# auniquesun/PPT

Measured on AMD Instinct MI355X. Metric: point-clouds/sec fwd+bwd, PointBERT 1024-pt ModelNet40, higher is better.
Workload: dtype f16; 1 GPU; C2: ModelNet40 1024-pt PointBERT (ULIP_PointBERT head_type=0, frozen backbone + PromptLearner), train-mode BN + DropPath, fwd + CE(ls 0.2) + bwd + AdamW; feed=resident, per_gpu_batch=32, global_batch=32, npoints=1024, classes=40, parallelism=dp1

## Files before the change

### include/ppt_hip.h

```cpp
#ifndef PPT_HIP_H
#define PPT_HIP_H

#include <stddef.h>
#include <stdint.h>

#ifdef __cplusplus
extern "C" {
#endif

#define PPT_OK 0
#define PPT_EINVAL (-1)
#define PPT_ELAUNCH (-2)
#define PPT_EUNSUPPORTED (-3)

#define PPT_F32 0
#define PPT_BF16 1
#define PPT_F16 2

const char *ppt_strerror(int code);
int ppt_abi_version(void);

int ppt_fps_f32(const float *xyz, int B, int N, int M, const int64_t *start, int64_t *out_idx,
                float *out_xyz, void *stream);

// ... 170 lines not shown
int ppt_text_mlp_retile_split(const float *W1, const float *W2, void *W1_tiled, void *W2_tiled, int b_pow2, void *stream);
int ppt_text_mlp_pair(const ppt_text_mlp_params *p, void *stream);

typedef struct ppt_text_lin_params {
    const void *A; int64_t lda;
    const void *W;
    const float *bias;
    const float *residual; int64_t ld_res;
    float *C; int64_t ldc;
    int M, N, K;
    int split_a_pow2, split_b_pow2; unsigned int *split_overflow;
    int wave_prio;
} ppt_text_lin_params;
int ppt_text_lin_retile_split(const float *W, void *W_tiled, int N, int K, int b_pow2, void *stream);
int ppt_text_lin_split(const ppt_text_lin_params *p, void *stream);

int ppt_attention_fwd(const void *qkv, void *out, float *lse, int Bt, int T, int H, int hd,
                      float scale, int causal, int dtype, void *stream);
int ppt_attention_bwd(const void *qkv, const void *out, const void *dout, const float *lse,
                      float *delta, void *dqkv, int Bt, int T, int H, int hd, float scale,
                      int causal, int dtype, void *stream);

size_t ppt_attention_prefix_workspace_bytes(int C, int P, int H, int hd);
int ppt_attention_fwd_split16(const void *qkv, void *out, float *lse, int Bt, int T, int P, int H, int hd, float scale, int causal,
                              void *stream);
int ppt_attention_bwd_split16(const void *qkv, const void *out, const void *dout, const float *lse, float *delta, void *dqkv,
                              float *workspace, int Bt, int T, int P, int H, int hd, float scale, int causal, void *stream);
int ppt_attention_prefix_fwd(const void *qkv, void *out, float *lse, int C, int T, int P, int H, int hd, float scale, int dtype,
                             void *stream);
int ppt_attention_prefix_bwd(const void *qkv, const void *out, const void *dout, const float *lse, float *delta, void *dqkv,
// ... 141 lines not shown
```

### ppt_amd/__init__.py

```python
import os

os.environ.setdefault("GPU_MAX_HW_QUEUES", "8")
```

### ppt_amd/_lib.py

```python
import ctypes
import os

_HERE = os.path.dirname(os.path.abspath(__file__))
LIB_PATH = os.environ.get("PPT_HIP_LIB") or os.path.join(_HERE, "csrc", "libppt_hip.so")
_lib = None

PPT_F32, PPT_BF16, PPT_F16 = 0, 1, 2
A_PLAIN, A_AFFINE_RELU, A_CONV1 = 0, 1, 2
ACT_NONE, ACT_RELU, ACT_GELU, ACT_QUICKGELU = 0, 1, 2, 3

c_void_p, c_int, c_int64, c_float, c_size_t = (ctypes.c_void_p, ctypes.c_int, ctypes.c_int64,
                                               ctypes.c_float, ctypes.c_size_t)


class GemmParams(ctypes.Structure):
    _fields_ = [
        ("A", c_void_p), ("lda", c_int64), ("B", c_void_p), ("ldb", c_int64),
        ("C", c_void_p), ("ldc", c_int64), ("M", c_int), ("N", c_int), ("K", c_int),
        ("dtype", c_int), ("c_dtype", c_int),
        ("a_mode", c_int), ("a_scale", c_void_p), ("a_shift", c_void_p), ("pts", c_void_p),
        ("w1", c_void_p), ("b1", c_void_p),
        ("bias", c_void_p), ("group_add", c_void_p), ("group_rows", c_int), ("act", c_int),
        ("dact_pre", c_void_p), ("ld_dact", c_int64),
        ("row_scale", c_void_p), ("row_scale_rows", c_int),
# ... 5 lines not shown
    ]


class LnLinParams(ctypes.Structure):
    _fields_ = [
        ("x", c_void_p), ("W", c_void_p), ("C", c_void_p), ("ln_w", c_void_p), ("ln_b", c_void_p), ("ln_eps", ctypes.c_float),
        ("bias", c_void_p), ("M", c_int), ("N", c_int), ("K", c_int), ("dtype", c_int), ("slices", c_int),
    ]


class TextLinParams(ctypes.Structure):
    _fields_ = [
        ("A", c_void_p), ("lda", c_int64), ("W", c_void_p), ("bias", c_void_p), ("residual", c_void_p), ("ld_res", c_int64),
        ("C", c_void_p), ("ldc", c_int64), ("M", c_int), ("N", c_int), ("K", c_int),
        ("split_a_pow2", c_int), ("split_b_pow2", c_int), ("split_overflow", c_void_p), ("wave_prio", c_int),
    ]


class TextMlpParams(ctypes.Structure):
    _fields_ = [
        ("A", c_void_p), ("lda", c_int64), ("W1", c_void_p), ("W2", c_void_p), ("b1", c_void_p), ("pre", c_void_p), ("parts", c_void_p),
        ("M", c_int), ("D", c_int), ("hidden", c_int), ("mode", c_int), ("dtype", c_int), ("wave_prio", c_int),
        ("ln_w", c_void_p), ("ln_b", c_void_p), ("ln_eps", ctypes.c_float), ("ln_mean", c_void_p), ("ln_rstd", c_void_p),
        ("split_a_pow2", c_int), ("split_b_pow2", c_int), ("split_overflow", c_void_p),
    ]


class VitMlpParams(ctypes.Structure):
    _fields_ = [
        ("x", c_void_p), ("out", c_void_p), ("W1", c_void_p), ("W2", c_void_p), ("ln_w", c_void_p), ("ln_b", c_void_p),
# ... 52 lines not shown
    "ppt_three_nn_interp_fwd": (c_int, [c_void_p, c_int, c_void_p, c_int, c_void_p, c_void_p, c_int, c_int, c_int, c_void_p, c_int,
                                        c_int, c_void_p, c_void_p]),
    "ppt_scatter_rows_bwd": (c_int, [c_void_p, c_void_p, c_void_p, c_int64, c_int, c_int, c_int, c_int, c_int, c_int, c_void_p,
                                     c_void_p]),
    "ppt_sum_groups": (c_int, [c_void_p, c_int64, c_int, c_int, c_void_p, c_void_p]),
    "ppt_vit_mlp_retile": (c_int, [c_void_p, c_void_p, c_void_p, c_void_p, c_void_p]),
    "ppt_vit_proj_retile": (c_int, [c_void_p, c_void_p, c_void_p]),
    "ppt_vit_mlp_bf16": (c_int, [ctypes.POINTER(VitMlpParams), c_void_p]),
    "ppt_lnlin_retile": (c_int, [c_void_p, c_void_p, c_int, c_void_p]),
    "ppt_lnlin": (c_int, [ctypes.POINTER(LnLinParams), c_void_p]),
    "ppt_text_mlp_retile": (c_int, [c_void_p, c_void_p, c_void_p, c_void_p, c_void_p]),
    "ppt_text_mlp_pair": (c_int, [ctypes.POINTER(TextMlpParams), c_void_p]),
    "ppt_text_mlp_retile_split": (c_int, [c_void_p, c_void_p, c_void_p, c_void_p, c_int, c_void_p]),
    "ppt_text_lin_retile_split": (c_int, [c_void_p, c_void_p, c_int, c_int, c_int, c_void_p]),
    "ppt_text_lin_split": (c_int, [ctypes.POINTER(TextLinParams), c_void_p]),
    "ppt_vit_mlp3_retile": (c_int, [c_void_p, c_void_p, c_void_p, c_void_p, c_void_p]),
    "ppt_vit_mlp3_bf16": (c_int, [ctypes.POINTER(VitMlpParams), c_void_p]),
    "ppt_rowgemm_bf16": (c_int, [ctypes.POINTER(RowGemmParams), c_void_p]),
    "ppt_layernorm_fwd": (c_int, [c_void_p, c_void_p, c_int, c_void_p, c_void_p, c_void_p, c_void_p, c_int,
                                  c_void_p, c_void_p, c_int, c_int, c_float, c_void_p]),
    "ppt_layernorm_bwd": (c_int, [c_void_p, c_void_p, c_void_p, c_void_p, c_void_p, c_void_p, c_int,
                                  c_void_p, c_int, c_void_p, c_void_p, c_int, c_int, c_int, c_void_p]),
    "ppt_layernorm_fwd_sum": (c_int, [c_void_p, c_void_p, c_void_p, c_int, c_void_p, c_void_p, c_void_p, c_void_p, c_int,
                                      c_void_p, c_void_p, c_int, c_int, c_float, c_void_p]),
    "ppt_layernorm_bwd_sum": (c_int, [c_void_p, c_int, c_void_p, c_void_p, c_void_p, c_void_p, c_void_p, c_int,
                                      c_void_p, c_int, c_int, c_int, c_void_p]),
    "ppt_col_sums": (c_int, [c_void_p, c_int, c_int, c_int, c_int64, c_void_p, c_void_p]),
    "ppt_attention_fwd": (c_int, [c_void_p, c_void_p, c_void_p, c_int, c_int, c_int, c_int, c_float, c_int,
                                  c_int, c_void_p]),
    "ppt_attention_bwd": (c_int, [c_void_p, c_void_p, c_void_p, c_void_p, c_void_p, c_void_p, c_int, c_int,
# ... 99 lines not shown
```

### ppt_amd/csrc/text_lin_split.hip

```cpp
#include "ppt_common.h"
#include "gemm_common.h"

namespace {

typedef __attribute__((ext_vector_type(4))) float f32x4_t;

constexpr int KC = 512;
constexpr int RB = 2, R = 16 * RB;
constexpr int AP = 2 * KC + 32;
constexpr int A_BYTES = R * AP;
constexpr int LDS_BYTES = 2 * A_BYTES;
constexpr int K1 = KC / 32;
constexpr int D1 = 4;

__device__ __forceinline__ void lds_barrier_l2()
{
    asm volatile("s_waitcnt lgkmcnt(0)" ::: "memory");
    __builtin_amdgcn_s_barrier();
    asm volatile("" ::: "memory");
}

__device__ __forceinline__ void split4_l(const float (&x)[4], uint2 &H, uint2 &L)
{
    uint32_t h[2], l[2];
#pragma unroll
    for (int q = 0; q < 2; ++q) {
        const _Float16 h0 = (_Float16)x[2 * q], h1 = (_Float16)x[2 * q + 1];
        const ppt_h2 hh = {h0, h1};
        const ppt_h2 ll = {(_Float16)(x[2 * q] - (float)h0), (_Float16)(x[2 * q + 1] - (float)h1)};
        h[q] = __builtin_bit_cast(uint32_t, hh);
        l[q] = __builtin_bit_cast(uint32_t, ll);
    }
    H = make_uint2(h[0], h[1]);
    L = make_uint2(l[0], l[1]);
}

template <int NH>
__global__ __launch_bounds__(512, 2) void text_lin_split_kernel(const ppt_text_lin_params p)
{
    constexpr int SLN = 128 * NH;
    constexpr int WAVE_SLICE = K1 * NH * 2048;
    extern __shared__ __align__(16) unsigned char smem[];
    unsigned char *ai = smem;
    const int lane = threadIdx.x & 63;
    const int w = __builtin_amdgcn_readfirstlane(threadIdx.x >> 6);
    const int l15 = lane & 15, kg = lane >> 4, lo16 = lane * 16;
    PPT_PRIO(p.wave_prio);
    const int nsl = p.N / SLN, nck = p.K / KC;
    const int sc = blockIdx.x % (nsl * nck), s = sc % nsl, c = sc / nsl;
    const int row0 = (blockIdx.x / (nsl * nck)) * R;
    const int nrow = min(R, p.M - row0);
    const float sa = pow2f(p.split_a_pow2), inv = pow2f(-(p.split_a_pow2 + p.split_b_pow2));
    uint32_t over = 0;

    const __amdgpu_buffer_rsrc_t r1 = __builtin_amdgcn_make_buffer_rsrc(const_cast<void *>(p.W), 0, (int)((size_t)p.N * p.K * 4), 0x00020000);
    int o1 = ((c * nsl + s) * 8 + w) * WAVE_SLICE;
    auto next1 = [&](uint4 (&f)[2 * NH]) {
#pragma unroll
        for (int i = 0; i < 2 * NH; ++i) f[i] = __builtin_bit_cast(uint4, __builtin_amdgcn_raw_buffer_load_b128(r1, lo16 + 1024 * i, o1, 0));
        o1 += 2048 * NH;
    };
    uint4 g1[D1][2 * NH];
#pragma unroll
    for (int i = 0; i < D1; ++i) next1(g1[i]);

    {
        const float *A = (const float *)p.A + (size_t)c * KC;
        constexpr int PIECES = R * (KC / 4);
        float4 v[PIECES / 512];
#pragma unroll
        for (int it = 0; it < PIECES / 512; ++it) {
            const int i = threadIdx.x + 512 * it, lr = i / (KC / 4), c4 = i % (KC / 4);
            v[it] = make_float4(0.f, 0.f, 0.f, 0.f);
            if (lr < nrow) v[it] = *reinterpret_cast<const float4 *>(A + (size_t)(row0 + lr) * p.lda + 4 * c4);
        }
#pragma unroll
        for (int it = 0; it < PIECES / 512; ++it) {
            const int i = threadIdx.x + 512 * it, lr = i / (KC / 4), c4 = i % (KC / 4);
            const float x[4] = {split_saturate(v[it].x * sa, over), split_saturate(v[it].y * sa, over),
                                split_saturate(v[it].z * sa, over), split_saturate(v[it].w * sa, over)};
            uint2 H, L;
            split4_l(x, H, L);
            *reinterpret_cast<uint2 *>(ai + lr * AP + 8 * c4) = H;
            *reinterpret_cast<uint2 *>(ai + A_BYTES + lr * AP + 8 * c4) = L;
        }
    }
    const int ncol = SLN * s + 16 * NH * w + 4 * kg;
    float4 bv[NH], rv[RB][NH];
#pragma unroll
    for (int h = 0; h < NH; ++h) {
        bv[h] = p.bias ? *reinterpret_cast<const float4 *>(p.bias + ncol + 16 * h) : make_float4(0.f, 0.f, 0.f, 0.f);
#pragma unroll
        for (int rb = 0; rb < RB; ++rb) {
            const int m = row0 + min(16 * rb + l15, nrow - 1);
            rv[rb][h] = p.residual ? *reinterpret_cast<const float4 *>(p.residual + (size_t)m * p.ld_res + ncol + 16 * h) : make_float4(0.f, 0.f, 0.f, 0.f);
        }
    }
    lds_barrier_l2();

    f32x4_t a1[RB][NH];
#pragma unroll
    for (int rb = 0; rb < RB; ++rb)
#pragma unroll
        for (int h = 0; h < NH; ++h) a1[rb][h] = f32x4_t{0.f, 0.f, 0.f, 0.f};
    {
        const unsigned char *ha = ai + l15 * AP + 16 * kg;
        uint4 fh[2][RB], fl[2][RB];
#pragma unroll
        for (int rb = 0; rb < RB; ++rb) {
            fh[0][rb] = *reinterpret_cast<const uint4 *>(ha + rb * 16 * AP);
            fl[0][rb] = *reinterpret_cast<const uint4 *>(ha + A_BYTES + rb * 16 * AP);
        }
#pragma unroll
        for (int ks = 0; ks < K1; ++ks) {
            if (ks + 1 < K1) {
#pragma unroll
                for (int rb = 0; rb < RB; ++rb) {
                    fh[(ks + 1) & 1][rb] = *reinterpret_cast<const uint4 *>(ha + rb * 16 * AP + 64 * (ks + 1));
                    fl[(ks + 1) & 1][rb] = *reinterpret_cast<const uint4 *>(ha + A_BYTES + rb * 16 * AP + 64 * (ks + 1));
                }
            }
#pragma unroll
            for (int h = 0; h < NH; ++h) {
                const uint4 wh = g1[ks % D1][2 * h], wl = g1[ks % D1][2 * h + 1];
#pragma unroll
                for (int rb = 0; rb < RB; ++rb) {
                    a1[rb][h] = h16<f16_t>::mfma16(wh, fl[ks & 1][rb], a1[rb][h]);
                    a1[rb][h] = h16<f16_t>::mfma16(wl, fh[ks & 1][rb], a1[rb][h]);
                    a1[rb][h] = h16<f16_t>::mfma16(wh, fh[ks & 1][rb], a1[rb][h]);
                }
            }
            if (ks + D1 < K1) next1(g1[ks % D1]);
            __builtin_amdgcn_sched_barrier(0);
        }
    }
    float *C = p.C + (size_t)c * p.M * p.ldc;
#pragma unroll
    for (int rb = 0; rb < RB; ++rb) {
        const int lr = 16 * rb + l15;
        if (lr < nrow) {
#pragma unroll
            for (int h = 0; h < NH; ++h)
                *reinterpret_cast<float4 *>(C + (size_t)(row0 + lr) * p.ldc + ncol + 16 * h) =
                    make_float4(a1[rb][h][0] * inv + bv[h].x + rv[rb][h].x, a1[rb][h][1] * inv + bv[h].y + rv[rb][h].y,
                                a1[rb][h][2] * inv + bv[h].z + rv[rb][h].z, a1[rb][h][3] * inv + bv[h].w + rv[rb][h].w);
        }
    }
    split_report(over, p.split_overflow);
}

template <int NH>
__global__ __launch_bounds__(256) void text_lin_retile_split_kernel(const float *__restrict__ W, unsigned char *__restrict__ Wt, int N, int K, int b_pow2)
{
    constexpr int SLN = 128 * NH;
    const int nsl = N / SLN, nck = K / KC;
    const int i = blockIdx.x * 256 + threadIdx.x;
    if (i >= nck * nsl * 8 * K1 * NH * 64) return;
    const int lane = i & 63, f = (i >> 6) % (K1 * NH), w = (i / (64 * K1 * NH)) & 7, sc = i / (64 * K1 * NH * 8);
    const int s = sc % nsl, c = sc / nsl, ks = f / NH, h = f % NH;
    const int l15 = lane & 15, kg = lane >> 4;
    const float sb = pow2f(b_pow2);
    const float *src = W + (size_t)(SLN * s + 16 * NH * w + 16 * h + l15) * K + KC * c + 32 * ks + 8 * kg;
    uint32_t over = 0;
    const float4 a = *reinterpret_cast<const float4 *>(src), b = *reinterpret_cast<const float4 *>(src + 4);
    const float x0[4] = {split_saturate(a.x * sb, over), split_saturate(a.y * sb, over), split_saturate(a.z * sb, over), split_saturate(a.w * sb, over)};
    const float x1[4] = {split_saturate(b.x * sb, over), split_saturate(b.y * sb, over), split_saturate(b.z * sb, over), split_saturate(b.w * sb, over)};
    uint2 h0, l0, h1, l1;
    split4_l(x0, h0, l0);
    split4_l(x1, h1, l1);
    unsigned char *dst = Wt + (size_t)(sc * 8 + w) * (K1 * NH * 2048) + (size_t)f * 2048 + lane * 16;
    *reinterpret_cast<uint4 *>(dst) = make_uint4(h0.x, h0.y, h1.x, h1.y);
    *reinterpret_cast<uint4 *>(dst + 1024) = make_uint4(l0.x, l0.y, l1.x, l1.y);
}

__host__ int slice_halves(int N) { return N >= 1024 ? 2 : 1; }

}

extern "C" int ppt_text_lin_retile_split(const float *W, void *Wt, int N, int K, int b_pow2, void *stream)
{
    if (!W || !Wt || (((uintptr_t)W | (uintptr_t)Wt) & 15) || abs(b_pow2) > 24) return PPT_EINVAL;
    if (N <= 0 || K <= 0 || K % KC || N % 256) return PPT_EUNSUPPORTED;
    const int pieces = N * (K / 8);
    if (slice_halves(N) == 2)
        hipLaunchKernelGGL(text_lin_retile_split_kernel<2>, dim3((pieces + 255) / 256), dim3(256), 0, ppt_stream(stream), W, (unsigned char *)Wt, N, K, b_pow2);
    else
        hipLaunchKernelGGL(text_lin_retile_split_kernel<1>, dim3((pieces + 255) / 256), dim3(256), 0, ppt_stream(stream), W, (unsigned char *)Wt, N, K, b_pow2);
    PPT_CHECK_LAUNCH();
    return PPT_OK;
}

extern "C" int ppt_text_lin_split(const ppt_text_lin_params *pp, void *stream)
{
    if (!pp) return PPT_EINVAL;
    ppt_text_lin_params p = *pp;
    if (!p.A || !p.W || !p.C || p.M <= 0 || p.N <= 0 || p.K <= 0) return PPT_EINVAL;
    if (p.K % KC || p.N % 256) return PPT_EUNSUPPORTED;
    if (p.lda < p.K || (p.lda % 4) || p.ldc < p.N || (p.ldc % 4) || abs(p.split_a_pow2) > 24 || abs(p.split_b_pow2) > 24) return PPT_EINVAL;
    if (((uintptr_t)p.A | (uintptr_t)p.W | (uintptr_t)p.C | (uintptr_t)p.bias | (uintptr_t)p.residual) & 15) return PPT_EINVAL;
    if (p.residual && (p.ld_res < p.N || (p.ld_res % 4))) return PPT_EINVAL;
    if (p.K > KC && (p.bias || p.residual || p.ldc != p.N)) return PPT_EINVAL;
    if (p.wave_prio == 0) p.wave_prio = ppt_get_wave_priority();
    static const int attrs_once = [] {
        (void)hipFuncSetAttribute((const void *)text_lin_split_kernel<1>, hipFuncAttributeMaxDynamicSharedMemorySize, LDS_BYTES);
        (void)hipFuncSetAttribute((const void *)text_lin_split_kernel<2>, hipFuncAttributeMaxDynamicSharedMemorySize, LDS_BYTES);
        return 0;
    }();
    (void)attrs_once;
    const int nh = slice_halves(p.N);
    const int grid = (p.N / (128 * nh)) * (p.K / KC) * ((p.M + R - 1) / R);
    hipStream_t st = ppt_stream(stream);
    if (nh == 2) hipLaunchKernelGGL((text_lin_split_kernel<2>), dim3(grid), dim3(512), LDS_BYTES, st, p);
    else hipLaunchKernelGGL((text_lin_split_kernel<1>), dim3(grid), dim3(512), LDS_BYTES, st, p);
    PPT_CHECK_LAUNCH();
    return PPT_OK;
}
```

### ppt_amd/engine.py

```python
import os

import torch

from . import ops
from .ops import ACT_GELU, ACT_NONE, ACT_QUICKGELU, A_AFFINE_RELU, A_CONV1

ATTN_SCALE = 64 ** -0.5


class WeightCache:

    def __init__(self, dtype, demoted=None):
        self.dtype = dtype
        self._c = {}
        self.demoted = demoted if demoted is not None else set()

    def get(self, t, kind="w", cols=None, pad_to=None):
        key = (id(t), kind, cols, pad_to)
        ent = self._c.get(key)
        if ent is not None and ent[0] is t and ent[1] == t._version:
            return ent[2]
        with torch.no_grad():
            w = t.detach()
            w = w.reshape(w.shape[0], -1)
# ... 669 lines not shown
TEXT_FUSE_LN = os.environ.get("PPT_TEXT_FUSE_LN", "0") != "0"
TEXT_SPLITK = os.environ.get("PPT_TEXT_SPLITK", "1") != "0"
POINTMLP_FUSED_NORM = os.environ.get("PPT_POINTMLP_FUSED_NORM", "1") != "0"


TEXT_MLP_PAIR = os.environ.get("PPT_TEXT_MLP_PAIR", "1") != "0"
TEXT_MLP_PAIR_LN = os.environ.get("PPT_TEXT_MLP_PAIR_LN", "1") != "0"
TEXT_MLP_PAIR_LAST = os.environ.get("PPT_TEXT_MLP_PAIR_LAST", "1") != "0"
TEXT_MLP_PAIR_SPLIT = os.environ.get("PPT_TEXT_MLP_PAIR_SPLIT", "1") != "0"


TEXT_LIN_SPLIT = os.environ.get("PPT_TEXT_LIN_SPLIT", "1") != "0"


def _text_lin_ok(Ta, width):
    return Ta == torch.float32 and TEXT_LIN_SPLIT and ops.split16_enabled() and width == 512


def _text_lin_tiles(sd, name, wca, transposed=False):
    w = sd[name]
    b = ops.SPLIT16_POW2[1]
    return wca.derived(("text_lin_split", name, transposed, b), (w,),
                       lambda: ops.text_lin_retile_split(wca.get(w, "wt") if transposed else wca.get(w), b))


def _text_mlp_pair_ok(Tm):
    return Tm in ops.HALF or (Tm == torch.float32 and TEXT_MLP_PAIR_SPLIT and ops.split16_enabled())


def _text_mlp_tiles(sd, p, wcm, backward):
    wfc, wpr = sd[p + "mlp.c_fc.weight"], sd[p + "mlp.c_proj.weight"]
    if wcm.dtype == torch.float32:
        b = ops.SPLIT16_POW2[1]
        if backward:
            return wcm.derived(("text_mlp_split_bwd", p, b), (wfc, wpr), lambda: ops.text_mlp_retile_split(wcm.get(wpr, "wt"), wcm.get(wfc, "wt"), b))
        return wcm.derived(("text_mlp_split_fwd", p, b), (wfc, wpr), lambda: ops.text_mlp_retile_split(wcm.get(wfc), wcm.get(wpr), b))
    if backward:
        return wcm.derived(("text_mlp_tiles_bwd", p), (wfc, wpr), lambda: ops.text_mlp_retile(wcm.get(wpr, "wt"), wcm.get(wfc, "wt")))
# ... 29 lines not shown
        M = C * L
        add, add_rows = sd["positional_embedding"], L
        xin = prompts.reshape(M, Wd)
        rows = torch.arange(C, device=dev) * L + eot_pos
    saved = {"layers": []} if save else None
    x = xin if add is None else torch.empty((M, Wd), dtype=torch.float32, device=dev)
    fuse = TEXT_FUSE_LN and T in ops.HALF and Wd in ops.ROWGEMM_K
    wca, wcm = _stage_wc(wc, "text_attn"), _stage_wc(wc, "text_mlp")
    Ta, Tm = wca.dtype, wcm.dtype
    if Ta != T or Tm != T:
        fuse = False

    def stats():
        return (torch.empty((M,), dtype=torch.float32, device=dev), torch.empty((M,), dtype=torch.float32, device=dev)) if save else None
    splitk = TEXT_SPLITK and (T in ops.HALF or ops.split16_enabled()) and Tm == T and not fuse and M <= 4096 and Wd == 512
    lin_split = _text_lin_ok(Ta, Wd) and not fuse
    pending = None
    for i in range(layers):
        p = f"transformer.resblocks.{i}."
        if pending is not None:
            x = torch.empty((M, Wd), dtype=torch.float32, device=dev)
            h, mean1, rstd1 = ops.layernorm_fwd_sum(pending[0], pending[1], pending[2], sd[p + "ln_1.weight"], sd[p + "ln_1.bias"], Ta,
                                                    write_xs=x, save_stats=save)
            pending = None
            if lin_split:
                qkv = ops.text_lin_split(h, _text_lin_tiles(sd, p + "attn.in_proj_weight", wca), bias=sd[p + "attn.in_proj_bias"])
            else:
                qkv = ops.gemm(h, wca.get(sd[p + "attn.in_proj_weight"]), out_dtype=Ta, bias=sd[p + "attn.in_proj_bias"])
        elif fuse and add is None:
            st1 = stats()
            mean1, rstd1 = st1 if save else (None, None)
            qkv = ops.rowgemm(xin, wc.get(sd[p + "attn.in_proj_weight"]), ln=(sd[p + "ln_1.weight"], sd[p + "ln_1.bias"]), ln_stats=st1,
                              bias=sd[p + "attn.in_proj_bias"])
        else:
            h, mean1, rstd1 = ops.layernorm_fwd(xin, sd[p + "ln_1.weight"], sd[p + "ln_1.bias"], Ta, add=add,
                                                add_rows=add_rows, write_xs=x if add is not None else None,
                                                save_stats=save)
            if lin_split:
                qkv = ops.text_lin_split(h, _text_lin_tiles(sd, p + "attn.in_proj_weight", wca), bias=sd[p + "attn.in_proj_bias"])
            else:
                qkv = ops.gemm(h, wca.get(sd[p + "attn.in_proj_weight"]), out_dtype=Ta, bias=sd[p + "attn.in_proj_bias"])
        add, add_rows = None, 0
        if P:
            a, lse = ops.attention_prefix_fwd(qkv, C, L, P, heads, ATTN_SCALE, want_lse=save)
        else:
            a, lse = ops.attention_fwd(qkv, C, L, heads, ATTN_SCALE, True, want_lse=save)
        x_mid = torch.empty_like(x)
        if lin_split:
            ops.text_lin_split(a, _text_lin_tiles(sd, p + "attn.out_proj.weight", wca), bias=sd[p + "attn.out_proj.bias"], residual=x, out=x_mid)
        else:
            ops.gemm(a, wca.get(sd[p + "attn.out_proj.weight"]), out=x_mid, bias=sd[p + "attn.out_proj.bias"], residual=x)
        pre = torch.empty((M, sd[p + "mlp.c_fc.weight"].shape[0]), dtype=Tm, device=dev) if save else None
        pair = (TEXT_MLP_PAIR and splitk and (i + 1 < layers or TEXT_MLP_PAIR_LAST) and _text_mlp_pair_ok(Tm)
                and tuple(sd[p + "mlp.c_fc.weight"].shape) == (2048, 512))
        if pair:
            w1t, w2t = _text_mlp_tiles(sd, p, wcm, False)
            if Tm == torch.float32 and TEXT_MLP_PAIR_LN:
                parts, mean2, rstd2 = ops.text_mlp_pair_split(x_mid, w1t, w2t, bias=sd[p + "mlp.c_fc.bias"], pre=pre,
                                                              ln=(sd[p + "ln_2.weight"], sd[p + "ln_2.bias"]), save_stats=save)
            elif Tm == torch.float32:
                h2, mean2, rstd2 = ops.layernorm_fwd(x_mid, sd[p + "ln_2.weight"], sd[p + "ln_2.bias"], Tm, save_stats=save)
                parts = ops.text_mlp_pair_split(h2, w1t, w2t, bias=sd[p + "mlp.c_fc.bias"], pre=pre)
            elif TEXT_MLP_PAIR_LN:
                parts, mean2, rstd2 = ops.text_mlp_pair(x_mid, w1t, w2t, bias=sd[p + "mlp.c_fc.bias"], pre=pre,
# ... 81 lines not shown
                                           sd[p + "ln_2.weight"], ly["mean2"], ly["rstd2"], g, accumulate=True, copy_dtype=Ta)
            d_pre = None
        else:
            d_pre = ops.gemm(g_t, wcm.get(sd[p + "mlp.c_proj.weight"], "wt"), out_dtype=Tm, act=ACT_QUICKGELU,
                             dact_pre=ly["pre"])
        if d_pre is None:
            pass
        elif splitk:
            _, g_t = ops.layernorm_bwd_sum(ops.gemm_splitk(d_pre, wcm.get(sd[p + "mlp.c_fc.weight"], "wt"), 4), ly["x_mid"],
                                           sd[p + "ln_2.weight"], ly["mean2"], ly["rstd2"], g, accumulate=True, copy_dtype=Ta)
        else:
            d_h2 = ops.gemm(d_pre, wcm.get(sd[p + "mlp.c_fc.weight"], "wt"), out_dtype=torch.float32)
            _, _, _, g_t = ops.layernorm_bwd(d_h2, ly["x_mid"], sd[p + "ln_2.weight"], ly["mean2"], ly["rstd2"], dx=g,
                                             accumulate=True, copy_dtype=Ta)
        if lin_split:
            d_a = ops.text_lin_split(g_t, _text_lin_tiles(sd, p + "attn.out_proj.weight", wca, True))
        else:
            d_a = ops.gemm(g_t, wca.get(sd[p + "attn.out_proj.weight"], "wt"), out_dtype=Ta)
        if P:
            d_qkv = ops.attention_prefix_bwd(ly["qkv"], ly["a"], d_a, ly["lse"], C, L, P, heads, ATTN_SCALE)
        else:
            d_qkv = ops.attention_bwd(ly["qkv"], ly["a"], d_a, ly["lse"], C, L, heads, ATTN_SCALE, True)
        if splitk:
            dparts = (ops.text_lin_split(d_qkv, _text_lin_tiles(sd, p + "attn.in_proj_weight", wca, True)) if lin_split
                      else ops.gemm_splitk(d_qkv, wca.get(sd[p + "attn.in_proj_weight"], "wt"), 3))
            _, g_t = ops.layernorm_bwd_sum(dparts, ly["x"],
                                           sd[p + "ln_1.weight"], ly["mean1"], ly["rstd1"], g, accumulate=True, copy_dtype=Tm)
        else:
            d_h = ops.gemm(d_qkv, wca.get(sd[p + "attn.in_proj_weight"], "wt"), out_dtype=torch.float32)
            _, _, _, g_t = ops.layernorm_bwd(d_h, ly["x"], sd[p + "ln_1.weight"], ly["mean1"], ly["rstd1"], dx=g,
                                             accumulate=True, copy_dtype=Tm)
    if s["rows_mode"]:
        return g
    if S != 1.0:
        g.mul_(1.0 / S)
    if not P and L == s["Lfull"]:
        return g.view(C, L, Wd)
    full = torch.zeros((C, s["Lfull"], Wd), dtype=torch.float32, device=dout.device)
    if P:
# ... 27 lines not shown
```

### ppt_amd/ops.py

```python
import ctypes
import os

import torch

from . import _lib
from ._lib import (ACT_GELU, ACT_NONE, ACT_QUICKGELU, ACT_RELU, A_AFFINE_RELU, A_CONV1, A_PLAIN,
                   PPT_BF16, PPT_F16, PPT_F32, GemmParams, RowGemmParams)
from . import _lib as _libmod

_DT = {torch.float32: PPT_F32, torch.bfloat16: PPT_BF16, torch.float16: PPT_F16}
_TORCH_DT = {PPT_F32: torch.float32, PPT_BF16: torch.bfloat16, PPT_F16: torch.float16}
HALF = (torch.bfloat16, torch.float16)


class KernelProfiler:

    def __init__(self):
        self.records = []
        self.kernels = []
        self.executed = []

    def begin(self, name, work, kernel=None, executed=None):
        ev = torch.cuda.Event(enable_timing=True)
        ev.record(torch.cuda.current_stream())
# ... 404 lines not shown
        p.residual, p.ld_res = _p(residual), residual.stride(-2)
    p.C, p.ldc = _p(out), (N if kc > 1 else out.stride(0))
    p.M, p.N, p.K = M, N, K
    p.split_a_pow2 = SPLIT16_POW2[0] if a_pow2 is None else int(a_pow2)
    p.split_b_pow2 = int(wt.ppt_b_pow2)
    if not torch.cuda.is_current_stream_capturing() or a.device.index in _SPLIT_OVERFLOW:
        p.split_overflow = _p(split16_overflow_counter(a.device))
    if profiler is not None:
        profiler.begin("gemm_f32", 2.0 * M * N * K, "ppt_text_lin_split")
    _lib.check(_lib.lib().ppt_text_lin_split(ctypes.byref(p), _stream()), "ppt_text_lin_split")
    if profiler is not None:
        profiler.end()
    return out


def text_mlp_pair(a, w1t, w2t, *, bias=None, pre=None, backward=False, ln=None, ln_eps=1e-5, save_stats=False):
    M = a.shape[0]
    assert a.dim() == 2 and a.shape[1] == 512 and a.stride(1) == 1 and w1t.dtype in HALF and w2t.dtype == w1t.dtype
    if ln is None:
        assert a.dtype == w1t.dtype
    else:
        assert a.dtype == torch.float32 and not backward
    parts = torch.empty((8, M, 512), dtype=torch.float32, device=a.device)
    p = _lib.TextMlpParams()
    p.A, p.lda, p.W1, p.W2, p.b1, p.pre, p.parts = _p(a), a.stride(0), _p(w1t), _p(w2t), _p(bias), _p(pre), _p(parts)
    p.M, p.D, p.hidden, p.mode, p.dtype = M, 512, 2048, int(bool(backward)), dtype_code(w1t)
    mean = rstd = None
    if ln is not None:
        _chk(ln[0], torch.float32, "ln weight"); _chk(ln[1], torch.float32, "ln bias")
        if save_stats:
# ... 771 lines not shown
```

Baseline: 11850 point-clouds/s.

## Add native half-precision text linear kernel path alongside split-f32 kernel

Generalizes the text-encoder linear kernel with a form template, so f16/bf16 activations and weights run a single MFMA per step. The split-f32 path needs two weight parts and three MFMAs per step. A new retile kernel and wrapper feed this path, and the engine routes half-precision text-encoder QKV and out-projection GEMMs (forward and backward) through it when split-K is active, replacing generic gemm calls. It also freezes the inherited GC heap in forked children. The half path drops split overflow tracking and relies on half-precision accuracy.

```diff
diff --git a/include/ppt_hip.h b/include/ppt_hip.h
--- a/include/ppt_hip.h
+++ b/include/ppt_hip.h
@@ -208,6 +208,19 @@
 } ppt_text_lin_params;
 int ppt_text_lin_retile_split(const float *W, void *W_tiled, int N, int K, int b_pow2, void *stream);
 int ppt_text_lin_split(const ppt_text_lin_params *p, void *stream);
+typedef struct ppt_text_lin16_params {
+    const void *A; int64_t lda;
+    const void *W;
+    const float *bias;
+    const float *residual; int64_t ld_res;
+    void *C; int64_t ldc;
+    int M, N, K;
+    int dtype;
+    int c_dtype;
+    int wave_prio;
+} ppt_text_lin16_params;
+int ppt_text_lin_retile16(const void *W, void *W_tiled, int N, int K, void *stream);
+int ppt_text_lin16(const ppt_text_lin16_params *p, void *stream);
 
 int ppt_attention_fwd(const void *qkv, void *out, float *lse, int Bt, int T, int H, int hd,
                       float scale, int causal, int dtype, void *stream);
diff --git a/ppt_amd/__init__.py b/ppt_amd/__init__.py
--- a/ppt_amd/__init__.py
+++ b/ppt_amd/__init__.py
@@ -1,3 +1,12 @@
 import os
 
 os.environ.setdefault("GPU_MAX_HW_QUEUES", "8")
+
+
+def _freeze_inherited_heap():
+    import gc
+    gc.freeze()
+
+
+if hasattr(os, "register_at_fork"):
+    os.register_at_fork(after_in_child=_freeze_inherited_heap)
diff --git a/ppt_amd/_lib.py b/ppt_amd/_lib.py
--- a/ppt_amd/_lib.py
+++ b/ppt_amd/_lib.py
@@ -43,6 +43,14 @@
         ("A", c_void_p), ("lda", c_int64), ("W", c_void_p), ("bias", c_void_p), ("residual", c_void_p), ("ld_res", c_int64),
         ("C", c_void_p), ("ldc", c_int64), ("M", c_int), ("N", c_int), ("K", c_int),
         ("split_a_pow2", c_int), ("split_b_pow2", c_int), ("split_overflow", c_void_p), ("wave_prio", c_int),
+    ]
+
+
+class TextLin16Params(ctypes.Structure):
+    _fields_ = [
+        ("A", c_void_p), ("lda", c_int64), ("W", c_void_p), ("bias", c_void_p), ("residual", c_void_p), ("ld_res", c_int64),
+        ("C", c_void_p), ("ldc", c_int64), ("M", c_int), ("N", c_int), ("K", c_int), ("dtype", c_int), ("c_dtype", c_int),
+        ("wave_prio", c_int),
     ]
 
 
@@ -125,6 +133,8 @@
     "ppt_text_mlp_retile_split": (c_int, [c_void_p, c_void_p, c_void_p, c_void_p, c_int, c_void_p]),
     "ppt_text_lin_retile_split": (c_int, [c_void_p, c_void_p, c_int, c_int, c_int, c_void_p]),
     "ppt_text_lin_split": (c_int, [ctypes.POINTER(TextLinParams), c_void_p]),
+    "ppt_text_lin_retile16": (c_int, [c_void_p, c_void_p, c_int, c_int, c_void_p]),
+    "ppt_text_lin16": (c_int, [ctypes.POINTER(TextLin16Params), c_void_p]),
     "ppt_vit_mlp3_retile": (c_int, [c_void_p, c_void_p, c_void_p, c_void_p, c_void_p]),
     "ppt_vit_mlp3_bf16": (c_int, [ctypes.POINTER(VitMlpParams), c_void_p]),
     "ppt_rowgemm_bf16": (c_int, [ctypes.POINTER(RowGemmParams), c_void_p]),
diff --git a/ppt_amd/csrc/text_lin_split.hip b/ppt_amd/csrc/text_lin_split.hip
--- a/ppt_amd/csrc/text_lin_split.hip
+++ b/ppt_amd/csrc/text_lin_split.hip
@@ -9,9 +9,32 @@
 constexpr int RB = 2, R = 16 * RB;
 constexpr int AP = 2 * KC + 32;
 constexpr int A_BYTES = R * AP;
-constexpr int LDS_BYTES = 2 * A_BYTES;
 constexpr int K1 = KC / 32;
-constexpr int D1 = 4;
+
+struct LinArgs {
+    const void *A; int64_t lda;
+    const void *W;
+    const float *bias;
+    const float *residual; int64_t ld_res;
+    void *C; int64_t ldc;
+    int M, N, K;
+    int c16;
+    int split_a_pow2, split_b_pow2; unsigned int *split_overflow;
+    int wave_prio;
+};
+
+template <int FORM> struct LinForm {
+    using T = typename std::conditional<FORM == PPT_BF16, bf16_t, f16_t>::type;
+    static constexpr bool SPLIT = false;
+    static constexpr int PARTS = 1;
+    static constexpr int D1 = 8;
+};
+template <> struct LinForm<PPT_F32> {
+    using T = f16_t;
+    static constexpr bool SPLIT = true;
+    static constexpr int PARTS = 2;
+    static constexpr int D1 = 4;
+};
 
 __device__ __forceinline__ void lds_barrier_l2()
 {
@@ -35,11 +58,13 @@
     L = make_uint2(l[0], l[1]);
 }
 
-template <int NH>
-__global__ __launch_bounds__(512, 2) void text_lin_split_kernel(const ppt_text_lin_params p)
-{
-    constexpr int SLN = 128 * NH;
-    constexpr int WAVE_SLICE = K1 * NH * 2048;
+template <int NH, int FORM>
+__global__ __launch_bounds__(512, 2) void text_lin_kernel(const LinArgs p)
+{
+    using F = LinForm<FORM>;
+    using T = typename F::T;
+    constexpr int SLN = 128 * NH, NP = F::PARTS * NH, D1 = F::D1;
+    constexpr int WAVE_SLICE = K1 * NP * 1024;
     extern __shared__ __align__(16) unsigned char smem[];
     unsigned char *ai = smem;
     const int lane = threadIdx.x & 63;
@@ -50,21 +75,32 @@
     const int sc = blockIdx.x % (nsl * nck), s = sc % nsl, c = sc / nsl;
     const int row0 = (blockIdx.x / (nsl * nck)) * R;
     const int nrow = min(R, p.M - row0);
-    const float sa = pow2f(p.split_a_pow2), inv = pow2f(-(p.split_a_pow2 + p.split_b_pow2));
     uint32_t over = 0;
 
-    const __amdgpu_buffer_rsrc_t r1 = __builtin_amdgcn_make_buffer_rsrc(const_cast<void *>(p.W), 0, (int)((size_t)p.N * p.K * 4), 0x00020000);
+    const __amdgpu_buffer_rsrc_t r1 = __builtin_amdgcn_make_buffer_rsrc(const_cast<void *>(p.W), 0, (int)((size_t)p.N * p.K * 2 * F::PARTS), 0x00020000);
     int o1 = ((c * nsl + s) * 8 + w) * WAVE_SLICE;
-    auto next1 = [&](uint4 (&f)[2 * NH]) {
-#pragma unroll
-        for (int i = 0; i < 2 * NH; ++i) f[i] = __builtin_bit_cast(uint4, __builtin_amdgcn_raw_buffer_load_b128(r1, lo16 + 1024 * i, o1, 0));
-        o1 += 2048 * NH;
+    auto next1 = [&](uint4 (&f)[NP]) {
+#pragma unroll
+        for (int i = 0; i < NP; ++i) f[i] = __builtin_bit_cast(uint4, __builtin_amdgcn_raw_buffer_load_b128(r1, lo16 + 1024 * i, o1, 0));
+        o1 += 1024 * NP;
     };
-    uint4 g1[D1][2 * NH];
+    constexpr int PIECES16 = R * (KC / 8);
+    uint4 v16[F::SPLIT ? 1 : PIECES16 / 512];
+    if constexpr (!F::SPLIT) {
+        const uint16_t *A = (const uint16_t *)p.A + (size_t)c * KC;
+#pragma unroll
+        for (int it = 0; it < PIECES16 / 512; ++it) {
+            const int i = threadIdx.x + 512 * it, lr = i / (KC / 8), c8 = i % (KC / 8);
+            v16[it] = make_uint4(0, 0, 0, 0);
+            if (lr < nrow) v16[it] = *reinterpret_cast<const uint4 *>(A + (size_t)(row0 + lr) * p.lda + 8 * c8);
+        }
+    }
+    uint4 g1[D1][NP];
 #pragma unroll
     for (int i = 0; i < D1; ++i) next1(g1[i]);
 
-    {
+    if constexpr (F::SPLIT) {
+        const float sa = pow2f(p.split_a_pow2);
         const float *A = (const float *)p.A + (size_t)c * KC;
         constexpr int PIECES = R * (KC / 4);
         float4 v[PIECES / 512];
@@ -84,6 +120,12 @@
             *reinterpret_cast<uint2 *>(ai + lr * AP + 8 * c4) = H;
             *reinterpret_cast<uint2 *>(ai + A_BYTES + lr * AP + 8 * c4) = L;
         }
+    } else {
+#pragma unroll
+        for (int it = 0; it < PIECES16 / 512; ++it) {
+            const int i = threadIdx.x + 512 * it, lr = i / (KC / 8), c8 = i % (KC / 8);
+            *reinterpret_cast<uint4 *>(ai + lr * AP + 16 * c8) = v16[it];
+        }
     }
     const int ncol = SLN * s + 16 * NH * w + 4 * kg;
     float4 bv[NH], rv[RB][NH];
@@ -109,7 +151,7 @@
 #pragma unroll
         for (int rb = 0; rb < RB; ++rb) {
             fh[0][rb] = *reinterpret_cast<const uint4 *>(ha + rb * 16 * AP);
-            fl[0][rb] = *reinterpret_cast<const uint4 *>(ha + A_BYTES + rb * 16 * AP);
+            if constexpr (F::SPLIT) fl[0][rb] = *reinterpret_cast<const uint4 *>(ha + A_BYTES + rb * 16 * AP);
         }
 #pragma unroll
         for (int ks = 0; ks < K1; ++ks) {
@@ -117,36 +159,51 @@
 #pragma unroll
                 for (int rb = 0; rb < RB; ++rb) {
                     fh[(ks + 1) & 1][rb] = *reinterpret_cast<const uint4 *>(ha + rb * 16 * AP + 64 * (ks + 1));
-                    fl[(ks + 1) & 1][rb] = *reinterpret_cast<const uint4 *>(ha + A_BYTES + rb * 16 * AP + 64 * (ks + 1));
+                    if constexpr (F::SPLIT) fl[(ks + 1) & 1][rb] = *reinterpret_cast<const uint4 *>(ha + A_BYTES + rb * 16 * AP + 64 * (ks + 1));
                 }
             }
 #pragma unroll
             for (int h = 0; h < NH; ++h) {
-                const uint4 wh = g1[ks % D1][2 * h], wl = g1[ks % D1][2 * h + 1];
-#pragma unroll
-                for (int rb = 0; rb < RB; ++rb) {
-                    a1[rb][h] = h16<f16_t>::mfma16(wh, fl[ks & 1][rb], a1[rb][h]);
-                    a1[rb][h] = h16<f16_t>::mfma16(wl, fh[ks & 1][rb], a1[rb][h]);
-                    a1[rb][h] = h16<f16_t>::mfma16(wh, fh[ks & 1][rb], a1[rb][h]);
+                if constexpr (F::SPLIT) {
+                    const uint4 wh = g1[ks % D1][2 * h], wl = g1[ks % D1][2 * h + 1];
+#pragma unroll
+                    for (int rb = 0; rb < RB; ++rb) {
+                        a1[rb][h] = h16<f16_t>::mfma16(wh, fl[ks & 1][rb], a1[rb][h]);
+                        a1[rb][h] = h16<f16_t>::mfma16(wl, fh[ks & 1][rb], a1[rb][h]);
+                        a1[rb][h] = h16<f16_t>::mfma16(wh, fh[ks & 1][rb], a1[rb][h]);
+                    }
+                } else {
+#pragma unroll
+                    for (int rb = 0; rb < RB; ++rb) a1[rb][h] = h16<T>::mfma16(g1[ks % D1][h], fh[ks & 1][rb], a1[rb][h]);
                 }
             }
             if (ks + D1 < K1) next1(g1[ks % D1]);
             __builtin_amdgcn_sched_barrier(0);
         }
     }
-    float *C = p.C + (size_t)c * p.M * p.ldc;
 #pragma unroll
     for (int rb = 0; rb < RB; ++rb) {
         const int lr = 16 * rb + l15;
         if (lr < nrow) {
 #pragma unroll
-            for (int h = 0; h < NH; ++h)
-                *reinterpret_cast<float4 *>(C + (size_t)(row0 + lr) * p.ldc + ncol + 16 * h) =
-                    make_float4(a1[rb][h][0] * inv + bv[h].x + rv[rb][h].x, a1[rb][h][1] * inv + bv[h].y + rv[rb][h].y,
-                                a1[rb][h][2] * inv + bv[h].z + rv[rb][h].z, a1[rb][h][3] * inv + bv[h].w + rv[rb][h].w);
-        }
-    }
-    split_report(over, p.split_overflow);
+            for (int h = 0; h < NH; ++h) {
+                if constexpr (F::SPLIT) {
+                    const float inv = pow2f(-(p.split_a_pow2 + p.split_b_pow2));
+                    float *C = (float *)p.C + (size_t)c * p.M * p.ldc;
+                    *reinterpret_cast<float4 *>(C + (size_t)(row0 + lr) * p.ldc + ncol + 16 * h) =
+                        make_float4(a1[rb][h][0] * inv + bv[h].x + rv[rb][h].x, a1[rb][h][1] * inv + bv[h].y + rv[rb][h].y,
+                                    a1[rb][h][2] * inv + bv[h].z + rv[rb][h].z, a1[rb][h][3] * inv + bv[h].w + rv[rb][h].w);
+                } else {
+                    const float4 v = make_float4(a1[rb][h][0] + bv[h].x + rv[rb][h].x, a1[rb][h][1] + bv[h].y + rv[rb][h].y,
+                                                 a1[rb][h][2] + bv[h].z + rv[rb][h].z, a1[rb][h][3] + bv[h].w + rv[rb][h].w);
+                    const size_t off = (size_t)c * p.M * p.ldc + (size_t)(row0 + lr) * p.ldc + ncol + 16 * h;
+                    if (p.c16) *reinterpret_cast<uint2 *>((uint16_t *)p.C + off) = make_uint2(h16<T>::pack2(v.x, v.y), h16<T>::pack2(v.z, v.w));
+                    else *reinterpret_cast<float4 *>((float *)p.C + off) = v;
+                }
+            }
+        }
+    }
+    if constexpr (F::SPLIT) split_report(over, p.split_overflow);
 }
 
 template <int NH>
@@ -173,7 +230,41 @@
     *reinterpret_cast<uint4 *>(dst + 1024) = make_uint4(l0.x, l0.y, l1.x, l1.y);
 }
 
+template <int NH>
+__global__ __launch_bounds__(256) void text_lin_retile16_kernel(const uint16_t *__restrict__ W, unsigned char *__restrict__ Wt, int N, int K)
+{
+    constexpr int SLN = 128 * NH;
+    const int nsl = N / SLN, nck = K / KC;
+    const int i = blockIdx.x * 256 + threadIdx.x;
+    if (i >= nck * nsl * 8 * K1 * NH * 64) return;
+    const int lane = i & 63, f = (i >> 6) % (K1 * NH), w = (i / (64 * K1 * NH)) & 7, sc = i / (64 * K1 * NH * 8);
+    const int s = sc % nsl, c = sc / nsl, ks = f / NH, h = f % NH;
+    const int l15 = lane & 15, kg = lane >> 4;
+    const uint16_t *src = W + (size_t)(SLN * s + 16 * NH * w + 16 * h + l15) * K + KC * c + 32 * ks + 8 * kg;
+    *reinterpret_cast<uint4 *>(Wt + (size_t)i * 16) = *reinterpret_cast<const uint4 *>(src);
+}
+
 __host__ int slice_halves(int N) { return N >= 1024 ? 2 : 1; }
+
+template <int NH, int FORM>
+void launch(const LinArgs &p, hipStream_t st)
+{
+    constexpr int LDS_BYTES = LinForm<FORM>::PARTS * A_BYTES;
+    static const int attrs_once = [] {
+        (void)hipFuncSetAttribute((const void *)text_lin_kernel<NH, FORM>, hipFuncAttributeMaxDynamicSharedMemorySize, LDS_BYTES);
+        return 0;
+    }();
+    (void)attrs_once;
+    const int grid = (p.N / (128 * NH)) * (p.K / KC) * ((p.M + R - 1) / R);
+    hipLaunchKernelGGL((text_lin_kernel<NH, FORM>), dim3(grid), dim3(512), LDS_BYTES, st, p);
+}
+
+template <int FORM>
+void launch_form(const LinArgs &p, hipStream_t st)
+{
+    if (slice_halves(p.N) == 2) launch<2, FORM>(p, st);
+    else launch<1, FORM>(p, st);
+}
 
 }
 
@@ -193,25 +284,50 @@
 extern "C" int ppt_text_lin_split(const ppt_text_lin_params *pp, void *stream)
 {
     if (!pp) return PPT_EINVAL;
-    ppt_text_lin_params p = *pp;
-    if (!p.A || !p.W || !p.C || p.M <= 0 || p.N <= 0 || p.K <= 0) return PPT_EINVAL;
-    if (p.K % KC || p.N % 256) return PPT_EUNSUPPORTED;
-    if (p.lda < p.K || (p.lda % 4) || p.ldc < p.N || (p.ldc % 4) || abs(p.split_a_pow2) > 24 || abs(p.split_b_pow2) > 24) return PPT_EINVAL;
-    if (((uintptr_t)p.A | (uintptr_t)p.W | (uintptr_t)p.C | (uintptr_t)p.bias | (uintptr_t)p.residual) & 15) return PPT_EINVAL;
-    if (p.residual && (p.ld_res < p.N || (p.ld_res % 4))) return PPT_EINVAL;
-    if (p.K > KC && (p.bias || p.residual || p.ldc != p.N)) return PPT_EINVAL;
-    if (p.wave_prio == 0) p.wave_prio = ppt_get_wave_priority();
-    static const int attrs_once = [] {
-        (void)hipFuncSetAttribute((const void *)text_lin_split_kernel<1>, hipFuncAttributeMaxDynamicSharedMemorySize, LDS_BYTES);
-        (void)hipFuncSetAttribute((const void *)text_lin_split_kernel<2>, hipFuncAttributeMaxDynamicSharedMemorySize, LDS_BYTES);
-        return 0;
-    }();
-    (void)attrs_once;
-    const int nh = slice_halves(p.N);
-    const int grid = (p.N / (128 * nh)) * (p.K / KC) * ((p.M + R - 1) / R);
-    hipStream_t st = ppt_stream(stream);
-    if (nh == 2) hipLaunchKernelGGL((text_lin_split_kernel<2>), dim3(grid), dim3(512), LDS_BYTES, st, p);
-    else hipLaunchKernelGGL((text_lin_split_kernel<1>), dim3(grid), dim3(512), LDS_BYTES, st, p);
+    const ppt_text_lin_params &q = *pp;
+    if (!q.A || !q.W || !q.C || q.M <= 0 || q.N <= 0 || q.K <= 0) return PPT_EINVAL;
+    if (q.K % KC || q.N % 256) return PPT_EUNSUPPORTED;
+    if (q.lda < q.K || (q.lda % 4) || q.ldc < q.N || (q.ldc % 4) || abs(q.split_a_pow2) > 24 || abs(q.split_b_pow2) > 24) return PPT_EINVAL;
+    if (((uintptr_t)q.A | (uintptr_t)q.W | (uintptr_t)q.C | (uintptr_t)q.bias | (uintptr_t)q.residual) & 15) return PPT_EINVAL;
+    if (q.residual && (q.ld_res < q.N || (q.ld_res % 4))) return PPT_EINVAL;
+    if (q.K > KC && (q.bias || q.residual || q.ldc != q.N)) return PPT_EINVAL;
+    const LinArgs p = {q.A, q.lda, q.W, q.bias, q.residual, q.ld_res, q.C, q.ldc, q.M, q.N, q.K, 0,
+                       q.split_a_pow2, q.split_b_pow2, q.split_overflow, q.wave_prio ? q.wave_prio : ppt_get_wave_priority()};
+    launch_form<PPT_F32>(p, ppt_stream(stream));
     PPT_CHECK_LAUNCH();
     return PPT_OK;
 }
+
+extern "C" int ppt_text_lin_retile16(const void *W, void *Wt, int N, int K, void *stream)
+{
+    if (!W || !Wt || (((uintptr_t)W | (uintptr_t)Wt) & 15)) return PPT_EINVAL;
+    if (N <= 0 || K <= 0 || K % KC || N % 256) return PPT_EUNSUPPORTED;
+    const int pieces = N * (K / 8);
+    if (slice_halves(N) == 2)
+        hipLaunchKernelGGL(text_lin_retile16_kernel<2>, dim3((pieces + 255) / 256), dim3(256), 0, ppt_stream(stream), (const uint16_t *)W, (unsigned char *)Wt, N, K);
+    else
+        hipLaunchKernelGGL(text_lin_retile16_kernel<1>, dim3((pieces + 255) / 256), dim3(256), 0, ppt_stream(stream), (const uint16_t *)W, (unsigned char *)Wt, N, K);
+    PPT_CHECK_LAUNCH();
+    return PPT_OK;
+}
+
+extern "C" int ppt_text_lin16(const ppt_text_lin16_params *pp, void *stream)
+{
+    if (!pp) return PPT_EINVAL;
+    const ppt_text_lin16_params &q = *pp;
+    if (!q.A || !q.W || !q.C || q.M <= 0 || q.N <= 0 || q.K <= 0) return PPT_EINVAL;
+    if (q.dtype != PPT_F16 && q.dtype != PPT_BF16) return PPT_EINVAL;
+    if (q.c_dtype != PPT_F32 && q.c_dtype != q.dtype) return PPT_EINVAL;
+    if (q.K % KC || q.N % 256) return PPT_EUNSUPPORTED;
+    if (q.lda < q.K || (q.lda % 8) || q.ldc < q.N || (q.ldc % 4)) return PPT_EINVAL;
+    if (((uintptr_t)q.A | (uintptr_t)q.W | (uintptr_t)q.bias | (uintptr_t)q.residual) & 15) return PPT_EINVAL;
+    if (((uintptr_t)q.C) & (q.c_dtype == PPT_F32 ? 15 : 7)) return PPT_EINVAL;
+    if (q.residual && (q.ld_res < q.N || (q.ld_res % 4))) return PPT_EINVAL;
+    if (q.K > KC && (q.bias || q.residual || q.ldc != q.N || q.c_dtype != PPT_F32)) return PPT_EINVAL;
+    const LinArgs p = {q.A, q.lda, q.W, q.bias, q.residual, q.ld_res, q.C, q.ldc, q.M, q.N, q.K, q.c_dtype != PPT_F32,
+                       0, 0, nullptr, q.wave_prio ? q.wave_prio : ppt_get_wave_priority()};
+    if (q.dtype == PPT_F16) launch_form<PPT_F16>(p, ppt_stream(stream));
+    else launch_form<PPT_BF16>(p, ppt_stream(stream));
+    PPT_CHECK_LAUNCH();
+    return PPT_OK;
+}
diff --git a/ppt_amd/engine.py b/ppt_amd/engine.py
--- a/ppt_amd/engine.py
+++ b/ppt_amd/engine.py
@@ -707,14 +707,22 @@
 
 
 def _text_lin_ok(Ta, width):
-    return Ta == torch.float32 and TEXT_LIN_SPLIT and ops.split16_enabled() and width == 512
+    return TEXT_LIN_SPLIT and width == 512 and (Ta in ops.HALF or (Ta == torch.float32 and ops.split16_enabled()))
 
 
 def _text_lin_tiles(sd, name, wca, transposed=False):
     w = sd[name]
+    if wca.dtype in ops.HALF:
+        return wca.derived(("text_lin16", name, transposed), (w,),
+                           lambda: ops.text_lin_retile16(wca.get(w, "wt") if transposed else wca.get(w)))
     b = ops.SPLIT16_POW2[1]
     return wca.derived(("text_lin_split", name, transposed, b), (w,),
                        lambda: ops.text_lin_retile_split(wca.get(w, "wt") if transposed else wca.get(w), b))
+
+
+def _text_lin(a, sd, name, wca, transposed=False, **kw):
+    wt = _text_lin_tiles(sd, name, wca, transposed)
+    return ops.text_lin16(a, wt, **kw) if wca.dtype in ops.HALF else ops.text_lin_split(a, wt, **kw)
 
 
 def _text_mlp_pair_ok(Tm):
@@ -774,7 +782,7 @@
     def stats():
         return (torch.empty((M,), dtype=torch.float32, device=dev), torch.empty((M,), dtype=torch.float32, device=dev)) if save else None
     splitk = TEXT_SPLITK and (T in ops.HALF or ops.split16_enabled()) and Tm == T and not fuse and M <= 4096 and Wd == 512
-    lin_split = _text_lin_ok(Ta, Wd) and not fuse
+    lin_split = _text_lin_ok(Ta, Wd) and not fuse and (Ta == torch.float32 or splitk)
     pending = None
     for i in range(layers):
         p = f"transformer.resblocks.{i}."
@@ -784,7 +792,7 @@
                                                     write_xs=x, save_stats=save)
             pending = None
             if lin_split:
-                qkv = ops.text_lin_split(h, _text_lin_tiles(sd, p + "attn.in_proj_weight", wca), bias=sd[p + "attn.in_proj_bias"])
+                qkv = _text_lin(h, sd, p + "attn.in_proj_weight", wca, bias=sd[p + "attn.in_proj_bias"])
             else:
                 qkv = ops.gemm(h, wca.get(sd[p + "attn.in_proj_weight"]), out_dtype=Ta, bias=sd[p + "attn.in_proj_bias"])
         elif fuse and add is None:
@@ -797,7 +805,7 @@
                                                 add_rows=add_rows, write_xs=x if add is not None else None,
                                                 save_stats=save)
             if lin_split:
-                qkv = ops.text_lin_split(h, _text_lin_tiles(sd, p + "attn.in_proj_weight", wca), bias=sd[p + "attn.in_proj_bias"])
+                qkv = _text_lin(h, sd, p + "attn.in_proj_weight", wca, bias=sd[p + "attn.in_proj_bias"])
             else:
                 qkv = ops.gemm(h, wca.get(sd[p + "attn.in_proj_weight"]), out_dtype=Ta, bias=sd[p + "attn.in_proj_bias"])
         add, add_rows = None, 0
@@ -807,7 +815,7 @@
             a, lse = ops.attention_fwd(qkv, C, L, heads, ATTN_SCALE, True, want_lse=save)
         x_mid = torch.empty_like(x)
         if lin_split:
-            ops.text_lin_split(a, _text_lin_tiles(sd, p + "attn.out_proj.weight", wca), bias=sd[p + "attn.out_proj.bias"], residual=x, out=x_mid)
+            _text_lin(a, sd, p + "attn.out_proj.weight", wca, bias=sd[p + "attn.out_proj.bias"], residual=x, out=x_mid)
         else:
             ops.gemm(a, wca.get(sd[p + "attn.out_proj.weight"]), out=x_mid, bias=sd[p + "attn.out_proj.bias"], residual=x)
         pre = torch.empty((M, sd[p + "mlp.c_fc.weight"].shape[0]), dtype=Tm, device=dev) if save else None
@@ -919,7 +927,7 @@
             _, _, _, g_t = ops.layernorm_bwd(d_h2, ly["x_mid"], sd[p + "ln_2.weight"], ly["mean2"], ly["rstd2"], dx=g,
                                              accumulate=True, copy_dtype=Ta)
         if lin_split:
-            d_a = ops.text_lin_split(g_t, _text_lin_tiles(sd, p + "attn.out_proj.weight", wca, True))
+            d_a = _text_lin(g_t, sd, p + "attn.out_proj.weight", wca, True)
         else:
             d_a = ops.gemm(g_t, wca.get(sd[p + "attn.out_proj.weight"], "wt"), out_dtype=Ta)
         if P:
@@ -927,7 +935,7 @@
         else:
             d_qkv = ops.attention_bwd(ly["qkv"], ly["a"], d_a, ly["lse"], C, L, heads, ATTN_SCALE, True)
         if splitk:
-            dparts = (ops.text_lin_split(d_qkv, _text_lin_tiles(sd, p + "attn.in_proj_weight", wca, True)) if lin_split
+            dparts = (_text_lin(d_qkv, sd, p + "attn.in_proj_weight", wca, True) if lin_split
                       else ops.gemm_splitk(d_qkv, wca.get(sd[p + "attn.in_proj_weight"], "wt"), 3))
             _, g_t = ops.layernorm_bwd_sum(dparts, ly["x"],
                                            sd[p + "ln_1.weight"], ly["mean1"], ly["rstd1"], g, accumulate=True, copy_dtype=Tm)
diff --git a/ppt_amd/ops.py b/ppt_amd/ops.py
--- a/ppt_amd/ops.py
+++ b/ppt_amd/ops.py
@@ -442,6 +442,42 @@
     return out
 
 
+def text_lin_retile16(w):
+    assert w.dtype in HALF and w.dim() == 2
+    _chk(w, w.dtype, "w")
+    N, K = w.shape
+    wt = torch.empty((N * K * 2,), dtype=torch.uint8, device=w.device)
+    _lib.check(_lib.lib().ppt_text_lin_retile16(_p(w), _p(wt), N, K, _stream()), "ppt_text_lin_retile16")
+    wt.ppt_shape, wt.ppt_dtype = (N, K), w.dtype
+    return wt
+
+
+def text_lin16(a, wt, *, bias=None, residual=None, out=None, out_dtype=None):
+    N, K = wt.ppt_shape
+    M = a.shape[0]
+    assert a.dtype == wt.ppt_dtype and a.dim() == 2 and a.shape[1] == K and a.stride(1) == 1
+    kc = K // 512
+    if kc > 1:
+        assert bias is None and residual is None and out is None and out_dtype in (None, torch.float32)
+        out = torch.empty((kc, M, N), dtype=torch.float32, device=a.device)
+    elif out is None:
+        out = torch.empty((M, N), dtype=out_dtype or a.dtype, device=a.device)
+    assert out.dtype in (torch.float32, a.dtype) and out.stride(-1) == 1
+    p = _lib.TextLin16Params()
+    p.A, p.lda, p.W, p.bias = _p(a), a.stride(0), _p(wt), _p(bias)
+    if residual is not None:
+        assert residual.dtype == torch.float32 and residual.stride(-1) == 1
+        p.residual, p.ld_res = _p(residual), residual.stride(-2)
+    p.C, p.ldc = _p(out), (N if kc > 1 else out.stride(0))
+    p.M, p.N, p.K, p.dtype, p.c_dtype = M, N, K, _DT[a.dtype], _DT[out.dtype]
+    if profiler is not None:
+        profiler.begin("gemm_bf16", 2.0 * M * N * K, "ppt_text_lin16")
+    _lib.check(_lib.lib().ppt_text_lin16(ctypes.byref(p), _stream()), "ppt_text_lin16")
+    if profiler is not None:
+        profiler.end()
+    return out
+
+
 def text_mlp_pair(a, w1t, w2t, *, bias=None, pre=None, backward=False, ln=None, ln_eps=1e-5, save_stats=False):
     M = a.shape[0]
     assert a.dim() == 2 and a.shape[1] == 512 and a.stride(1) == 1 and w1t.dtype in HALF and w2t.dtype == w1t.dtype
```

Measured after the change: 12190 point-clouds/s, median of 6. +2.8%, better.
